# JialeTao/MRFA

Hardware: AMD Instinct MI355X
Metric: frames/sec (256x256 source+driving pair) fwd+bwd (higher is better)
Workload: dtype f32; 1 GPU; vox1.yaml MTIA (TokenPose_B) prior + DenseMotion + RaftFlow refinement, 256x256, bs=8/GPU, fwd+bwd+clip+Adam, train-mode BN, surrogate L1 loss; global_batch=8, parallelism=dp1, prior=mtia, background_predictor=False, sync_bn=False, launch=hipGraph, optimizer=FlatAdam (K20), mfma=bf16x6

## Files before the change

### mrfa_amd/build.py

```python
import glob
import os
import subprocess
import sys

HERE = os.path.dirname(os.path.abspath(__file__))
ROOT = os.path.dirname(HERE)
CSRC = os.path.join(HERE, "csrc")
LIBDIR = os.path.join(HERE, "_lib")
LIB = os.path.join(LIBDIR, "libmrfa_hip.so")
SOURCES = ["error.cpp", "conv_plan.hip", "conv_mfma.hip", "conv_split.hip", "conv_halo.hip", "conv_small.hip", "conv_lean.hip", "wgrad_mfma.hip", "wgrad_split.hip", "wgrad_halo.hip", "wgrad_small.hip", "wgrad_lean.hip", "conv_fewout.hip", "conv_fewout3.hip", "layout.hip", "pack_multi.hip", "norm.hip", "sample.hip", "elementwise.hip", "optim.hip", "tokenpose.hip", "attention_mfma.hip", "losses.hip", "prior.hip"]
FLAGS = ["--offload-arch=gfx950", "-O3", "-std=c++17", "-fPIC", "-I" + os.path.join(ROOT, "include"), "-I" + CSRC,
         "-Wno-unused-result"]


def _stale(out, deps):
    if not os.path.exists(out):
        return True
    t = os.path.getmtime(out)
    return any(os.path.getmtime(d) > t for d in deps)


def build(force: bool = False, verbose: bool = True) -> str:
    os.makedirs(LIBDIR, exist_ok=True)
    hipcc = os.environ.get("HIPCC", "/opt/rocm/bin/hipcc")
    headers = [os.path.join(ROOT, "include", "mrfa_hip.h")] + sorted(glob.glob(os.path.join(CSRC, "*.h")))
    objs = []
    procs = []
    for src in SOURCES:
        sp = os.path.join(CSRC, src)
        if not os.path.exists(sp):
            raise FileNotFoundError(sp)
        obj = os.path.join(LIBDIR, os.path.splitext(src)[0] + ".o")
        objs.append(obj)
        if force or _stale(obj, [sp] + headers):
            cmd = [hipcc] + FLAGS + (["-x", "hip"] if src.endswith(".cpp") else []) + ["-c", sp, "-o", obj]
            if verbose:
                print("[mrfa_amd.build]", " ".join(cmd), flush=True)
            procs.append((src, subprocess.Popen(cmd)))
    for src, pr in procs:
        if pr.wait() != 0:
            raise RuntimeError(f"hipcc failed on {src}")
    if force or _stale(LIB, objs):
        cmd = [hipcc, "--offload-arch=gfx950", "-shared", "-fPIC", "-o", LIB] + objs
        if verbose:
            print("[mrfa_amd.build]", " ".join(cmd), flush=True)
        subprocess.check_call(cmd)
    return LIB


if __name__ == "__main__":
    build(force="--force" in sys.argv)
    print(LIB)
```

### mrfa_amd/csrc/common.h

```cpp
#pragma once
#include <hip/hip_runtime.h>
#include <stdio.h>
#include <string.h>
#include "mrfa_hip.h"

typedef float f32x16 __attribute__((ext_vector_type(16)));
typedef float f32x4 __attribute__((ext_vector_type(4)));

void mrfa_set_error(const char* fmt, ...);

struct MrfaTuning {
    int conv_small_env;
    int conv_small;
    int conv_halo, conv_halo_min_tiles, conv_halo_pr, conv_halo_phase, conv_halo_bn256, conv_halo_bn192, conv_halo_bn64_fill;
    int conv_lean, conv_lean_min_wgs, conv_lean_geo, gemm_lean;
    int wgrad_halo, wgrad_halo_min_wgs, wgrad_halo_target_wgs, wgrad_halo_phase, wgrad_lean;
    int conv_fewout3, attention_mfma, split_target_256;
};
extern MrfaTuning g_tune;

struct HaloGeo { int PR, BN; bool phase; };

enum class ConvFamily { lean, gemm_lean, small, halo, halo_dgrad, rows_split, rows_f32, refused };
struct ConvPlan {
    ConvFamily family;
    char error[256];
    long long M;
    int KT;
    int lean_geo, gemm_cfg, small_tm, small_tn;
    HaloGeo halo;
    int BM, BN, splitk;
    bool w8;
    bool fused;
    bool fin_in_launch;
    bool reads_w;
    int last_config;
    bool groups_ok, bst_ok, stride2_ok, mask_ok, phase_dgrad_ok;
};
ConvPlan plan_conv(const mrfa_conv_params& p);

enum class WgradFamily { lean, small, halo, tiled, refused };
struct WgradPlan {
    WgradFamily family;
    char error[192];
    long long M;
    bool lean, small;
    bool groups_ok, stride2_ok;
};
WgradPlan plan_wgrad(const mrfa_wgrad_params& p);

int mrfa_conv_split_launch(hipStream_t st, const mrfa_conv_params& p, int KT, long long M, int splitk, int BN);
bool mrfa_conv_halo_eligible(const mrfa_conv_params& p, HaloGeo* geo);
int mrfa_conv_halo_launch(hipStream_t st, const mrfa_conv_params& p, const HaloGeo& geo);
int mrfa_wgrad_split_launch(hipStream_t st, const mrfa_wgrad_params& p, dim3 grid, long long M, long long kps, int tiles_n, int nsplit, int inner,
                            int total_splits, int taps, long long partial_stride, int BM, int BN);

bool mrfa_wgrad_halo_eligible(const mrfa_wgrad_params& p);
int mrfa_wgrad_halo_launch(hipStream_t st, const mrfa_wgrad_params& p);

bool mrfa_fewout3_wgrad(hipStream_t st, const float* x, int ldx, int N, int H, int W, int Cin, const float* dy, int lddy, int Cout, int R, int pad,
                        float* dw, float* dbias, int* rc);

int mrfa_conv_lean_pick(const mrfa_conv_params& p);
int mrfa_conv_lean_launch(hipStream_t st, const mrfa_conv_params& p, int geo);
int mrfa_gemm_lean_pick(const mrfa_conv_params& p, long long M);
int mrfa_gemm_lean_launch(hipStream_t st, const mrfa_conv_params& p, long long M, int cfg);

bool mrfa_conv_small_eligible(const mrfa_conv_params& p, long long M);
int mrfa_conv_small_launch(hipStream_t st, const mrfa_conv_params& p, long long M, int tm, int tn);

bool mrfa_attention_mfma_ok(int d, int n, const void* qkv, int ld, const void* out, int ldo, const void* dout, int lddo, const void* dqkv, int lddq);
int mrfa_attention_fwd_mfma(hipStream_t st, const float* qkv, int ld, int B, int n, int heads, int d, float scale, float* out, int ldo, float* lse);
int mrfa_attention_bwd_mfma(hipStream_t st, const float* qkv, int ld, const float* out, int ldo, const float* dout, int lddo, const float* lse,
                            float* delta, int B, int n, int heads, int d, float scale, float* dqkv, int lddq);

bool mrfa_wgrad_lean_eligible(const mrfa_wgrad_params& p);
int mrfa_wgrad_lean_multi(hipStream_t st, const mrfa_wgrad_params* ps, int n, unsigned char* taken);

bool mrfa_wgrad_small_eligible(const mrfa_wgrad_params& p, long long M);
int mrfa_wgrad_small_launch(hipStream_t st, const mrfa_wgrad_params& p, long long M);

#define MRFA_CHECK_ARG(cond, ...)                      \
    do {                                               \
        if (!(cond)) {                                 \
            mrfa_set_error(__VA_ARGS__);               \
            return 1;                                  \
        }                                              \
    } while (0)

#define MRFA_CHECK_LAUNCH(name)                                                   \
    do {                                                                          \
        hipError_t e_ = hipGetLastError();                                        \
        if (e_ != hipSuccess) {                                                   \
            mrfa_set_error("%s: launch failed: %s", name, hipGetErrorString(e_)); \
            return 2;                                                             \
        }                                                                         \
    } while (0)

static inline bool aligned16(const void* p) { return (reinterpret_cast<uintptr_t>(p) & 15u) == 0; }
static inline int cdiv(long long a, long long b) { return (int)((a + b - 1) / b); }

static inline int stream_grid(long long work_items, int block) {
    long long g = (work_items + block - 1) / block;
    if (g < 1) g = 1;
    if (g > 256 * 16) g = 256 * 16;
    return (int)g;
}

__device__ __forceinline__ int xcd_tile_index() {
    const int per_xcd = (int)gridDim.x >> 3;
    return (int)(blockIdx.x & 7) * per_xcd + (int)(blockIdx.x >> 3);
}

__device__ __forceinline__ void chain_prio() {
    __builtin_amdgcn_s_setprio(3);
}

__device__ __forceinline__ int stat_group(const mrfa_conv_params& p, long long row, long long M) {
    return p.groups > 1 ? (int)(row / (M / p.groups)) : 0;
}
__device__ __forceinline__ double* stat_slot(const mrfa_conv_params& p, int group, unsigned slot) {
    return p.stats + ((size_t)group * MRFA_STATS_SLOTS + slot % MRFA_STATS_SLOTS) * 2 * p.Cout;
}
static inline long long group_rows(const mrfa_conv_params& p, long long M) {
    if (p.groups <= 1) return M;
    return (p.N % p.groups) == 0 ? M / p.groups : 0;
}

__device__ __forceinline__ bool splitk_last_arriver(unsigned* ticket, unsigned nsplit) {
    __shared__ unsigned s_sk_ticket;
    asm volatile("s_waitcnt vmcnt(0)" ::: "memory");
    __syncthreads();
    if (threadIdx.x == 0) s_sk_ticket = __hip_atomic_fetch_add(ticket, 1u, __ATOMIC_RELAXED, __HIP_MEMORY_SCOPE_AGENT);
    __syncthreads();
    return s_sk_ticket == nsplit - 1;
}

__device__ __forceinline__ bool fin_last_arriver(unsigned* counter, unsigned participants, int idx) {
    __shared__ unsigned s_fin_ticket;
    asm volatile("s_waitcnt vmcnt(0)" ::: "memory");
    __syncthreads();
    if (threadIdx.x == 0) {
        if (idx < 0) {
            s_fin_ticket = __hip_atomic_fetch_add(counter, 1u, __ATOMIC_RELAXED, __HIP_MEMORY_SCOPE_AGENT) == participants - 1;
// ... 63 lines not shown
```

### mrfa_amd/csrc/conv_fewout.hip

```cpp
#include "common.h"

namespace {

constexpr int FT = 16;
constexpr int FCC = 16;
constexpr int FPS = FCC + 4;

template <int COUT, int PY, int RT>
__global__ __launch_bounds__(256) void conv_fewout_fwd_kernel(const float* __restrict__ x, int ldx, int H, int W, int Cin,
                                                             const float* __restrict__ w, const float* __restrict__ bias,
                                                             float* __restrict__ y, int ldy, int Ho, int Wo, int Rdyn, int pad,
                                                             int accumulate, int tiles_x, int tiles_y, int cper) {
    extern __shared__ __attribute__((aligned(16))) float smem[];
    const int R = RT > 0 ? RT : Rdyn;
    const int HTW = FT + R - 1, HTH = FT * PY + R - 1;
    const int tid = threadIdx.x;
    const int tx = tid & 15, ty = tid >> 4;
    const int bt = blockIdx.x;
    const int n = bt / (tiles_x * tiles_y);
    const int trem = bt - n * tiles_x * tiles_y;
    const int ty0 = (trem / tiles_x) * FT * PY, tx0 = (trem % tiles_x) * FT;
    const int T = R * R;
    float acc[PY][COUT];
#pragma unroll
// ... 145 lines not shown
                    const float* xrow = xs + ((py + r) * HT + s) * ps + g4 * 4;
                    const float* drow = dys + py * FT * 4;
#pragma unroll 4
                    for (int pxx = 0; pxx < FT; ++pxx) {
                        const f32x4 xv = *reinterpret_cast<const f32x4*>(xrow + pxx * ps);
                        const f32x4 dv = *reinterpret_cast<const f32x4*>(drow + pxx * 4);
#pragma unroll
                        for (int c = 0; c < COUT; ++c) acc[c] += xv * dv[c];
                    }
                }
            }
            if (dbias && c0 == 0 && tid < COUT) {
                float sacc = 0.f;
                for (int q = 0; q < 256; ++q) sacc += dys[q * 4 + tid];
                bsum += sacc;
            }
        }
        if (active) {
#pragma unroll
            for (int c = 0; c < COUT; ++c) {
                float* d = dw + ((size_t)c * T + tap) * Cin + c0 + g4 * 4;
#pragma unroll
                for (int q = 0; q < 4; ++q)
                    if (c0 + g4 * 4 + q < Cin) atomicAdd(d + q, acc[c][q]);
            }
        }
        if (dbias && c0 == 0 && tid < COUT) atomicAdd(dbias + tid, bsum);
    }
}

}

extern "C" int mrfa_conv_fewout_fwd(void* stream, const float* x, int ldx, int N, int H, int W, int Cin, const float* w,
                                    const float* bias, float* y, int ldy, int Cout, int R, int pad, int accumulate) {
    MRFA_CHECK_ARG(x && w && y && Cout >= 1 && Cout <= 4 && (Cin % 4) == 0 && (ldx % 4) == 0 && aligned16(x) && aligned16(w),
                   "conv_fewout_fwd: needs Cout <= 4, Cin %% 4 == 0, 16-B aligned x / w");
    const int Ho = H + 2 * pad - R + 1, Wo = W + 2 * pad - R + 1;
    const int PY = (R >= 5 && Cout <= 2 && Ho >= 32) ? 2 : 1;
    const bool rt7 = true;
    const int tiles_x = cdiv(Wo, FT), tiles_y = cdiv(Ho, FT * PY);
    const size_t lds = (size_t)(FT * PY + R - 1) * (FT + R - 1) * FPS * sizeof(float);
    if (lds > 64 * 1024) {
        MRFA_CHECK_ARG(lds <= 160 * 1024, "conv_fewout_fwd: halo tile does not fit the LDS");
    }
    hipStream_t st = (hipStream_t)stream;
    const int ntiles = N * tiles_x * tiles_y;
    const int chunks = cdiv(Cin, FCC);
    const int want = 1024;
    int csplit = 1;
    if (ntiles < want / 2 && chunks > 1) {
        csplit = cdiv(want, ntiles);
        if (csplit > chunks) csplit = chunks;
    }
    const int cper = cdiv(chunks, csplit) * FCC;
    csplit = cdiv(Cin, cper);
    if (csplit > 1 && !accumulate) {
        const long long tot = (long long)N * Ho * Wo * Cout;
        hipLaunchKernelGGL(fewout_init_kernel, dim3((unsigned)cdiv(tot, 256)), dim3(256), 0, st, y, ldy, (long long)N * Ho * Wo, Cout, bias);
    }
    dim3 grid((unsigned)ntiles, (unsigned)csplit);
#define FWD3(co, py, rt)                                                                                                                        \
    do {                                                                                                                                    \
        if (lds > 64 * 1024)                                                                                                                \
            (void)hipFuncSetAttribute(reinterpret_cast<const void*>(conv_fewout_fwd_kernel<co, py, rt>), hipFuncAttributeMaxDynamicSharedMemorySize, (int)lds); \
        hipLaunchKernelGGL((conv_fewout_fwd_kernel<co, py, rt>), grid, dim3(256), lds, st, x, ldx, H, W, Cin, w, bias, y, ldy, Ho, Wo, R, pad,   \
                           accumulate, tiles_x, tiles_y, cper);                                                                             \
    } while (0)
#define FWD2(co, py) do { if (R == 7 && rt7) FWD3(co, py, 7); else FWD3(co, py, 0); } while (0)
#define FWD(co) do { if (PY == 4) FWD2(co, 4); else if (PY == 2) FWD2(co, 2); else FWD2(co, 1); } while (0)
    switch (Cout) { case 1: FWD(1); break; case 2: FWD(2); break; case 3: FWD(3); break; default: FWD(4); break; }
#undef FWD
#undef FWD2
#undef FWD3
    MRFA_CHECK_LAUNCH("conv_fewout_fwd");
    return 0;
}

extern "C" int mrfa_conv_fewout_wgrad(void* stream, const float* x, int ldx, int N, int H, int W, int Cin, const float* dy, int lddy,
                                      int Cout, int R, int pad, float* dw, float* dbias) {
    MRFA_CHECK_ARG(x && dy && dw && Cout >= 1 && Cout <= 4 && (Cin % 4) == 0 && (ldx % 4) == 0 && aligned16(x),
                   "conv_fewout_wgrad: needs Cout <= 4, Cin %% 4 == 0, 16-B aligned x");
    {
        int rc3 = 0;
        if (mrfa_fewout3_wgrad((hipStream_t)stream, x, ldx, N, H, W, Cin, dy, lddy, Cout, R, pad, dw, dbias, &rc3)) return rc3;
    }
    const int Ho = H + 2 * pad - R + 1, Wo = W + 2 * pad - R + 1;
    const int tiles_x = cdiv(Wo, FT), tiles_y = cdiv(Ho, FT);
    const int ntiles = N * tiles_x * tiles_y;
    const int T = R * R;
    MRFA_CHECK_ARG(T * 1 <= 256, "conv_fewout_wgrad: kernel too large");
    int cc = 4;
    const int HT = FT + R - 1;
    auto lds_of = [&](int c) { return ((size_t)HT * HT * (c + 4) + 256 * 4) * sizeof(float); };
    const int cc_max = ntiles < 64 ? 16 : 64;
    while (cc * 2 <= cc_max && T * (cc * 2 / 4) <= 256 && cc * 2 <= ((Cin + 3) / 4 * 4) && lds_of(cc * 2) <= 64 * 1024) cc *= 2;
    const size_t lds = lds_of(cc);
    MRFA_CHECK_ARG(lds <= 64 * 1024, "conv_fewout_wgrad: LDS tile too large");
    dim3 grid((unsigned)(ntiles < 512 ? ntiles : 512), (unsigned)cdiv(Cin, cc));
    hipStream_t st = (hipStream_t)stream;
#define WG(co) hipLaunchKernelGGL((conv_fewout_wgrad_kernel<co>), grid, dim3(256), lds, st, x, ldx, H, W, Cin, dy, lddy, Ho, Wo, R, pad, dw, \
                                  dbias, tiles_x, tiles_y, ntiles, cc)
    switch (Cout) { case 1: WG(1); break; case 2: WG(2); break; case 3: WG(3); break; default: WG(4); break; }
#undef WG
    MRFA_CHECK_LAUNCH("conv_fewout_wgrad");
    return 0;
}
```

### mrfa_amd/csrc/conv_plan.hip

```cpp
#include "common.h"
#include <stdarg.h>
#include <stdlib.h>

namespace {
int env_int(const char* name, int dflt) { const char* e = getenv(name); return e ? atoi(e) : dflt; }
int env_on(const char* name) { const char* e = getenv(name); return !(e && e[0] == '0'); }
}

MrfaTuning g_tune = {
     env_on("MRFA_CONV_SMALL"),  1,
     env_on("MRFA_CONV_HALO"),  128,  0,  1,  1,
     1,  1,
     env_on("MRFA_CONV_LEAN"),  128,  -1,
     env_int("MRFA_GEMM_LEAN", 1),
     env_on("MRFA_WGRAD_HALO"),  192,  256,  1,
     env_on("MRFA_WGRAD_LEAN"),
     1,  env_on("MRFA_ATTENTION_MFMA"),  env_int("MRFA_SPLIT_TARGET_256", 1),
};

enum TuneKind { T_ON, T_INT, T_NONNEG, T_NONNEG_ON, T_LEVEL, T_POS };
static const struct { const char* key; int* field; TuneKind kind; } TUNING_KEYS[] = {
    {"conv_small", &g_tune.conv_small, T_ON},
    {"conv_halo", &g_tune.conv_halo, T_ON},
    {"conv_halo_min_tiles", &g_tune.conv_halo_min_tiles, T_INT},
    {"conv_halo_pr", &g_tune.conv_halo_pr, T_INT},
    {"conv_halo_phase", &g_tune.conv_halo_phase, T_ON},
    {"conv_halo_bn256", &g_tune.conv_halo_bn256, T_ON},
    {"conv_halo_bn192", &g_tune.conv_halo_bn192, T_ON},
    {"conv_halo_bn64_fill", &g_tune.conv_halo_bn64_fill, T_ON},
    {"conv_lean", &g_tune.conv_lean, T_ON},
    {"conv_lean_min_wgs", &g_tune.conv_lean_min_wgs, T_NONNEG},
    {"conv_lean_geo", &g_tune.conv_lean_geo, T_INT},
    {"gemm_lean", &g_tune.gemm_lean, T_LEVEL},
    {"wgrad_halo", &g_tune.wgrad_halo, T_ON},
    {"wgrad_halo_min_wgs", &g_tune.wgrad_halo_min_wgs, T_NONNEG},
    {"wgrad_halo_target_wgs", &g_tune.wgrad_halo_target_wgs, T_POS},
    {"wgrad_halo_phase", &g_tune.wgrad_halo_phase, T_NONNEG_ON},
    {"wgrad_lean", &g_tune.wgrad_lean, T_ON},
    {"conv_fewout3", &g_tune.conv_fewout3, T_ON},
    {"attention_mfma", &g_tune.attention_mfma, T_ON},
};

extern "C" int mrfa_set_tuning(const char* key, int value) {
    if (!key) return -1;
    for (const auto& k : TUNING_KEYS) {
        if (strcmp(key, k.key)) continue;
        const int prev = *k.field;
        switch (k.kind) {
            case T_ON: *k.field = value != 0; break;
            case T_INT: *k.field = value; break;
            case T_NONNEG: if (value >= 0) *k.field = value; break;
            case T_NONNEG_ON: if (value >= 0) *k.field = value != 0; break;
            case T_LEVEL: if (value >= 0) *k.field = value > 2 ? 2 : value; break;
            case T_POS: if (value > 0) *k.field = value; break;
        }
        return prev;
    }
    return -1;
}

namespace {
constexpr int BK = 32;

template <typename Plan>
Plan& refuse(Plan& c, const char* fmt, ...) {
    va_list ap;
    va_start(ap, fmt);
    vsnprintf(c.error, sizeof(c.error), fmt, ap);
    va_end(ap);
    c.family = decltype(c.family)::refused;
    return c;
}

void plan_rows(ConvPlan& c, const mrfa_conv_params& p, int mode) {
    const bool flat = p.kflat > 0;
    const long long M = c.M;
    const int KT = c.KT;
    const int nb = p.nbatch > 1 ? p.nbatch : 1;
    int BN = 128;
    {
        const int cands[4] = {128, 96, 64, 32};
        const double pen[4] = {1.0, 1.08, 1.16, 1.3};
        double best = 1e18;
        for (int i = 0; i < 4; ++i) {
            if (cands[i] == 96 && flat) continue;
            const double cost = (double)cdiv(p.Cout, cands[i]) * cands[i] * pen[i];
            if (cost < best) { best = cost; BN = cands[i]; }
        }
    }
    if (mode >= 1 && !flat && p.Cout >= 32) BN = p.Cout <= 64 ? 64 : 128;
    auto ntiles = [&](int bm, int bn) { return ((M + bm - 1) / bm) * cdiv(p.Cout, bn) * nb; };
    int BM = 128;
    if (BN == 96 && ntiles(128, 96) < 384) BN = 128;
    if (BN == 128) { if (M <= 32) BM = 32; else if (M <= 64) BM = 64; }
    else if (BN == 64 && M <= 64) BM = 64;
    int splitk = 1;
    const bool auto_split = (p.splitk == 0);
    if (p.splitk > 1) splitk = p.splitk;
    {
        const bool short_k_big_m = KT < 32 && M > 4096;
        const bool grouped_stats = p.groups > 1 && p.stats && !(p.sk_ticket && !p.accumulate);
        const int max_split = (auto_split && !short_k_big_m && !grouped_stats) ? (KT / 2 > 0 ? KT / 2 : 1) : 1;
        long long t = ntiles(BM, BN);
        if (t < 384 && !(short_k_big_m && t >= 128)) {
            const bool half_target = g_tune.split_target_256 && auto_split && p.sk_ticket && !p.accumulate && KT >= 72 && KT <= 320 && BM == 128 && t >= 8 && t <= 16;
            int want = (int)(((half_target ? 256 : 512) + t - 1) / t);
            if (auto_split) splitk = want <= max_split ? want : max_split;
            const int min_bm = (BN == 128) ? 32 : (BN == 64 ? 64 : 128);
            while (!half_target && ntiles(BM, BN) * splitk < 384 && BM > min_bm) {
                BM >>= 1;
                if (auto_split) {
                    t = ntiles(BM, BN);
                    want = (int)((512 + t - 1) / t);
                    splitk = want <= max_split ? want : max_split;
                }
            }
            if (splitk < 1) splitk = 1;
        }
    }
    bool w8 = false;
    if (p.tile) {
        BM = p.tile >> 16; BN = p.tile & 0x7fff; w8 = (p.tile & 0x8000) != 0;
// ... 23 lines not shown
    c.splitk = 1;
    c.reads_w = true;
    c.fin_in_launch = p.fin_scale != nullptr;

    c.lean_geo = flat ? -1 : mrfa_conv_lean_pick(p);
    c.gemm_cfg = (flat || c.lean_geo >= 0) ? -1 : mrfa_gemm_lean_pick(p, c.M);
    const bool lean = c.lean_geo >= 0, gemm = c.gemm_cfg >= 0;
    const bool small = !lean && !gemm && g_tune.conv_small_env && g_tune.conv_small && mrfa_conv_small_eligible(p, c.M);
    const bool halo = !flat && mrfa_conv_halo_eligible(p, &c.halo);

    const long long rows = group_rows(p, c.M);
    c.groups_ok = p.groups <= 1 || !(p.stats || p.fin_scale || p.bst_x || p.in_scale) ||
                  (p.nbatch <= 1 && p.splitk <= 1 && rows > 0 &&
                   (lean || gemm || (!p.in_scale && ((rows % 128) == 0 || small || (p.stride <= 1 && halo)))));
    c.bst_ok = p.stats && !p.fin_scale && p.stride >= 0 && !flat && (lean || gemm || small);
    c.stride2_ok = p.stride == 2 && p.Hout == (p.Hin + 2 * p.pad - p.R) / 2 + 1 && p.Wout == (p.Win + 2 * p.pad - p.S) / 2 + 1 &&
                   (flat ? (!p.ups && p.nbatch <= 1 && p.splitk <= 1 && p.ktab) : small);
    c.mask_ok = halo;
    c.phase_dgrad_ok = p.ups == 2 && halo;

    if (!(p.x && p.w)) return refuse(c, "conv2d: null pointer");
    if (!(p.N > 0 && p.Cin > 0 && p.Cout > 0 && p.Hout > 0 && p.Wout > 0)) return refuse(c, "conv2d: bad sizes");
    if (!(p.R >= 1 && p.S >= 1 && p.R <= 15 && p.S <= 15)) return refuse(c, "conv2d: kernel size %dx%d unsupported", p.R, p.S);
    if (!((p.w_ld % 4) == 0 && aligned16(p.w))) return refuse(c, "conv2d: packed weight must be 16-B aligned, w_ld %% 4 == 0");
    if (!flat && (p.Cin % 32) != 0) return refuse(c, "conv2d: chunked mode needs Cin %% 32 == 0 (got %d); use flat mode", p.Cin);
    if (!flat && !((p.ldx % 4) == 0 && aligned16(p.x))) return refuse(c, "conv2d: chunked mode needs 16-B aligned x and ldx %% 4 == 0");
    if (!flat && p.in_scale && !(aligned16(p.in_scale) && aligned16(p.in_shift))) return refuse(c, "conv2d: in_scale/in_shift alignment");
    if (flat && !(p.ktab != nullptr && aligned16(p.ktab))) return refuse(c, "conv2d: flat mode needs a 16-B aligned ktab");
    if (lean) {
        c.family = ConvFamily::lean;
        c.reads_w = false;
        c.last_config = (32 << 16) | (32 << 4) | 4 | (1 << 27);
        return c;
    }
    if (gemm) {
        c.family = ConvFamily::gemm_lean;
        c.reads_w = false;
        c.last_config = (64 << 16) | (64 << 4) | 4 | (1 << 26);
        return c;
    }
    if (small) {
        c.family = ConvFamily::small;
        const int ncols = (p.Cout + 15) / 16 * 16;
        auto waves = [&](int wm, int wn) { return ((c.M + wm - 1) / wm) * ((ncols + wn - 1) / wn); };
        int tm = 2, tn = 2;
        if (waves(32, 32) < 2048) { tm = 1; tn = 2; }
        if (tm == 1 && waves(16, 32) < 2048) { tn = 1; }
        if (ncols % 32 != 0 && tn == 2 && ncols < 32) tn = 1;
        if (p.groups > 1 && tm == 2 && (rows % 128) != 0) tm = 1;
        c.small_tm = tm;
        c.small_tn = tn;
        c.last_config = (16 << 16) | (16 << 4) | 8;
        return c;
    }
    if (p.stride < 0 || p.stride > 2 || (p.stride == 2 && !(flat && !p.ups && p.nbatch <= 1)))
        return refuse(c, "conv2d: stride = %d is only implemented by the one-wave-per-tile kernel and by flat-K launches: ask mrfa_conv2d_stride_supported() first", p.stride);
    if (p.mask && !halo) return refuse(c, "conv2d: `mask` is only honoured by the patch-tiled kernel: ask mrfa_conv2d_mask_supported() first");
    if (p.ups == 2 && !halo)
        return refuse(c, "conv2d: ups = 2 (phase data gradient of a fused-upsample layer) is only implemented for the shapes mrfa_conv2d_phase_dgrad_supported() reports");
    if (halo) {
        c.family = p.ups == 2 ? ConvFamily::halo_dgrad : ConvFamily::halo;
        c.reads_w = false;
        c.last_config = (128 << 16) | ((p.Cout <= 64 ? 64 : 128) << 4) | 4 | (1 << 28);
        return c;
    }
    plan_rows(c, p, mode);
    return c;
}

WgradPlan plan_wgrad(const mrfa_wgrad_params& p) {
    WgradPlan c = {};
    const bool flat = p.kflat > 0;
    c.M = (long long)p.N * p.Hout * p.Wout;
    c.lean = mrfa_wgrad_lean_eligible(p);
    c.small = g_tune.conv_small_env && g_tune.conv_small && mrfa_wgrad_small_eligible(p, c.M);
    c.groups_ok = p.groups <= 1 || !p.in_scale || c.lean;
    c.stride2_ok = p.stride == 2 && p.Hout == (p.Hin + 2 * p.pad - p.R) / 2 + 1 && p.Wout == (p.Win + 2 * p.pad - p.S) / 2 + 1 && c.small;
    if (!(p.x && p.dy && p.dw)) return refuse(c, "wgrad: null pointer");
    if (!flat && !((p.ldx % 4) == 0 && aligned16(p.x))) return refuse(c, "wgrad: x must be a 16-B aligned view with ld %% 4 == 0");
    if (flat && !p.ktab) return refuse(c, "wgrad: flat mode needs ktab");
    if (!(c.M < (1ll << 31) - 64)) return refuse(c, "wgrad: too many pixels");
    if (p.in_scale && c.lean) { c.family = WgradFamily::lean; return c; }
    if (!c.groups_ok) return refuse(c, "wgrad: groups = %d with a prologue is only implemented where mrfa_conv2d_wgrad_groups_supported() says so", p.groups);
    if (c.small) { c.family = WgradFamily::small; return c; }
    if (p.stride > 1) return refuse(c, "wgrad: stride = %d is only implemented by the small-problem kernel: ask mrfa_conv2d_wgrad_stride_supported() first", p.stride);
    c.family = !flat && mrfa_wgrad_halo_eligible(p) ? WgradFamily::halo : WgradFamily::tiled;
    return c;
}

extern "C" int mrfa_conv2d_split_k(const mrfa_conv_params* p) {
    if (!p) return 1;
    if (p->splitk > 1) return p->splitk;
    const ConvPlan c = plan_conv(*p);
    return c.family == ConvFamily::refused ? 1 : c.splitk;
}

extern "C" int mrfa_conv2d_reads_fp32_weights(const mrfa_conv_params* p) {
    if (!p) return 1;
    const ConvPlan c = plan_conv(*p);
    return c.family == ConvFamily::refused || c.reads_w ? 1 : 0;
}

extern "C" int mrfa_conv2d_groups_supported(const mrfa_conv_params* p) { return p && plan_conv(*p).groups_ok ? 1 : 0; }
extern "C" int mrfa_conv2d_bwdstats_supported(const mrfa_conv_params* p) { return p && plan_conv(*p).bst_ok ? 1 : 0; }
extern "C" int mrfa_conv2d_stride_supported(const mrfa_conv_params* p) { return p && plan_conv(*p).stride2_ok ? 1 : 0; }
extern "C" int mrfa_conv2d_mask_supported(const mrfa_conv_params* p) { return p && plan_conv(*p).mask_ok ? 1 : 0; }
extern "C" int mrfa_conv2d_phase_dgrad_supported(const mrfa_conv_params* p) { return p && plan_conv(*p).phase_dgrad_ok ? 1 : 0; }

extern "C" int mrfa_conv2d_wgrad_stride_supported(const mrfa_wgrad_params* p) { return p && plan_wgrad(*p).stride2_ok ? 1 : 0; }
extern "C" int mrfa_conv2d_wgrad_groups_supported(const mrfa_wgrad_params* p) { return p && plan_wgrad(*p).groups_ok ? 1 : 0; }
extern "C" int mrfa_conv2d_wgrad_lean_supported(const mrfa_wgrad_params* p) { return p && plan_wgrad(*p).lean ? 1 : 0; }
```

### mrfa_amd/csrc/wgrad_mfma.hip

```cpp
#include "common.h"
#include <stdlib.h>
#include <algorithm>

namespace {

constexpr int WBK = 32;
constexpr int KG = WBK / 4;

template <int BM, int BN, int WAVES_M, int WAVES_N, bool FLAT, bool ROWAL>
__global__ __launch_bounds__(WAVES_M * WAVES_N * 64) void wgrad_mfma_kernel(const mrfa_wgrad_params p, const long long M, const long long k_per_split,
                                                        const int tiles_n, const int nsplit, const int dy_scalar,
                                                        const int inner, const int total_splits, const int taps,
                                                        const long long partial_stride) {
    constexpr int WTM = BM / WAVES_M, WTN = BN / WAVES_N;
    constexpr int TM = WTM / 32, TN = WTN / 32;
    constexpr int NT = WAVES_M * WAVES_N * 64;
    static_assert((NT == 256 || NT == 512) && TM >= 1 && TN >= 1, "tile");
    constexpr int SA = BM / 4 + 4, SB = BN / 4 + 4;
    constexpr int PLA = 4 * SA, PLB = 4 * SB;
    constexpr int IA = (BM / 4) * KG, IB = (BN / 4) * KG;
    __shared__ f32x4 smem[2 * KG * (PLA + PLB)];

    const int tid = threadIdx.x, lane = tid & 63, wave = tid >> 6;
    const int wm = wave / WAVES_N, wn = wave % WAVES_N;
// ... 235 lines not shown
        const f32x4* Bs = smem + cur * KG * (PLA + PLB) + KG * PLA + b_lane;
#pragma unroll
        for (int q = 0; q < KG / 2; ++q) {
            f32x4 a[TM], b[TN];
#pragma unroll
            for (int i = 0; i < TM; ++i) a[i] = As[(2 * q + fh) * PLA + i * 8];
#pragma unroll
            for (int j = 0; j < TN; ++j) b[j] = Bs[(2 * q + fh) * PLB + j * 8];
#pragma unroll
            for (int e = 0; e < 4; ++e)
#pragma unroll
                for (int i = 0; i < TM; ++i)
#pragma unroll
                    for (int j = 0; j < TN; ++j)
                        acc[i][j] = __builtin_amdgcn_mfma_f32_32x32x2f32(a[i][e], b[j][e], acc[i][j], 0, 0, 0);
        }
        if (more) store_tiles(cur ^ 1);
        __syncthreads();
        cur ^= 1;
    }

#pragma unroll
    for (int j = 0; j < TN; ++j) {
        const int nn = ci0 + wn * WTN + j * 32 + (lane & 31);
        if (nn >= NTOT) continue;
        const int otap = FLAT ? nn / p.Cin : tap;
        const int ci = FLAT ? nn - otap * p.Cin : nn;
#pragma unroll
        for (int i = 0; i < TM; ++i) {
#pragma unroll
            for (int q = 0; q < 16; ++q) {
                const int co = co0 + wm * WTM + i * 32 + (q & 3) + 8 * (q >> 2) + 4 * fh;
                if (co < p.Cout) {
                    const size_t idx = ((size_t)otap * p.Cout + co) * p.Cin + ci;
                    if (partial_stride) p.ws[(size_t)split * partial_stride + idx] = acc[i][j][q] * p.alpha;
                    else atomicAdd(dw + idx, acc[i][j][q] * p.alpha);
                }
            }
        }
    }
    if (p.dbias != nullptr && tap == 0 && tile_n == 0) {
        float* red = reinterpret_cast<float*>(smem);
        __syncthreads();
        if (a_item) {
#pragma unroll
            for (int q = 0; q < 4; ++q) red[a_kg * BM + a_col + q] = bias_acc[q];
        }
        __syncthreads();
        if (tid < BM && co0 + tid < p.Cout) {
            float sacc = 0.f;
#pragma unroll
            for (int g = 0; g < KG; ++g) sacc += red[g * BM + tid];
            atomicAdd(p.dbias + co0 + tid, sacc);
        }
    }
}


__global__ void wgrad_reduce_kernel(const float* __restrict__ ws, float* __restrict__ dw, long long n, int nsplit) {
    const int groups = (nsplit + 15) / 16;
    const long long total = n * groups;
    for (long long t = blockIdx.x * (long long)blockDim.x + threadIdx.x; t < total; t += (long long)gridDim.x * blockDim.x) {
        const int g = (int)(t / n);
        const long long i = t - (long long)g * n;
        const int k0 = g * 16, k1 = min(nsplit, k0 + 16);
        float s = 0.f;
#pragma unroll 16
        for (int k = k0; k < k1; ++k) s += ws[(size_t)k * n + i];
        atomicAdd(dw + i, s);
    }
}

}

extern "C" int mrfa_conv2d_wgrad_nhwc(void* stream, const mrfa_wgrad_params* pp) {
    const mrfa_wgrad_params& p = *pp;
    hipStream_t st = (hipStream_t)stream;
    const WgradPlan c = plan_wgrad(p);
    const long long M = c.M;
    switch (c.family) {
        case WgradFamily::refused: mrfa_set_error("%s", c.error); return 1;
        case WgradFamily::lean: { unsigned char taken = 0; return mrfa_wgrad_lean_multi(st, &p, 1, &taken); }
        case WgradFamily::small: return mrfa_wgrad_small_launch(st, p, M);
        case WgradFamily::halo: return mrfa_wgrad_halo_launch(st, p);
        case WgradFamily::tiled: break;
    }
    const int dy_scalar = ((p.ldy % 4) == 0 && aligned16(p.dy) && (p.dy_bs % 4) == 0) ? 0 : 1;
    const bool flat = p.kflat > 0;
    const int nb = p.nbatch > 1 ? p.nbatch : 1;
    int taps = flat ? 1 : p.R * p.S;
    const int NTOT = flat ? p.kflat : p.Cin;
    auto pick = [](int n) {
        const int cands[4] = {128, 96, 64, 32};
        const double pen[4] = {1.0, 1.12, 1.35, 1.8};
        int best_t = 128;
        double best = 1e18;
        for (int i = 0; i < 4; ++i) {
            const double cost = (double)cdiv(n, cands[i]) * cands[i] * pen[i];
            if (cost < best) { best = cost; best_t = cands[i]; }
        }
        return best_t;
    };
    int BM = pick(p.Cout), BN = pick(NTOT);
    if (BM < 128 && BN < 128) {
        if (BM == 64 && BN == 64) {}
        else if (BM <= BN) BN = 128;
        else BM = 128;
    }
    if (flat && (BM == 96 || BN == 96)) { BM = BM == 96 ? 128 : BM; BN = BN == 96 ? 128 : BN; }
    const bool split_mode = mrfa_get_mfma_mode() >= 1 && !flat && (p.Wout % 8) == 0 && (M % WBK) == 0 && !dy_scalar && p.Cout >= 32 && NTOT >= 32;
    if (split_mode) { BM = p.Cout <= 64 ? 64 : 128; BN = NTOT <= 64 ? 64 : 128; if (BM == 64 && BN == 64) BN = 128; }
    int tiles_m = cdiv(p.Cout, BM), tiles_n = cdiv(NTOT, BN);
    int taps_arg = taps;
    constexpr bool cflat_on = true;
    if (cflat_on && split_mode && taps > 1 && (p.Cin % 4) == 0) {
        const double per_tap = (double)taps * tiles_n * BN * (BN == 64 ? 1.4 : 1.0), flat_w = (double)cdiv(taps * p.Cin, 128) * 128;
        if (flat_w <= 0.85 * per_tap) {
            BN = 128;
            tiles_n = cdiv(taps * p.Cin, 128);
            taps = 1;
            taps_arg = -1;
        }
    }
    const long long base = (long long)tiles_m * tiles_n * taps * nb;
    int nsplit = p.ksplit;
    if (nsplit <= 0) {
        const long long max_split = std::max<long long>(1, M / (8 * WBK));
        double best = 1e30;
        nsplit = 1;
        const long long inner_ = (long long)tiles_m * tiles_n * taps;
        for (long long ns = 1; ns <= std::min<long long>(max_split, 1024); ++ns) {
            const long long S = ns * nb;
            const long long ktiles = ((M + ns - 1) / ns + WBK - 1) / WBK;
            double rounds;
            if (S >= 8) rounds = (double)(((S + 7) / 8 * inner_ + 63) / 64);
            else rounds = (double)((S * inner_ + 511) / 512);
            const double cost = rounds * (double)(ktiles + 6);
            if (cost < best * 0.999) { best = cost; nsplit = (int)ns; }
        }
    }
    long long kps = (M + nsplit - 1) / nsplit;
    kps = (kps + WBK - 1) / WBK * WBK;
    nsplit = (int)((M + kps - 1) / kps);
    const int inner = tiles_m * tiles_n * taps;
    const int total_splits = nsplit * nb;
    const long long wn = (long long)(flat ? 1 : taps) * 0 + (long long)p.R * p.S * p.Cout * p.Cin;
    const long long partial_stride = (nb == 1 && nsplit >= 24 && p.ws && wn * nsplit * 4 <= p.ws_bytes) ? wn : 0;
    dim3 grid((unsigned)(cdiv(total_splits, 8) * 8 * inner));
    const bool rowal = (p.Wout % WBK) == 0;
#define WLAUNCH(bm, bn, wm, wn, fl, ra)                                                                                     \
    hipLaunchKernelGGL((wgrad_mfma_kernel<bm, bn, wm, wn, fl, ra>), grid, dim3((wm) * (wn) * 64), 0, st, p, M, kps, tiles_n, nsplit, dy_scalar, \
                       inner, total_splits, taps, partial_stride)
#define WCFG(bm, bn, wm, wn)                                              \
    if (BM == bm && BN == bn) {                                           \
        if (flat && rowal) WLAUNCH(bm, bn, wm, wn, true, true);           \
        else if (flat) WLAUNCH(bm, bn, wm, wn, true, false);              \
        else if (rowal) WLAUNCH(bm, bn, wm, wn, false, true);             \
        else WLAUNCH(bm, bn, wm, wn, false, false);                       \
    }
    if (split_mode) {
        const int rc = mrfa_wgrad_split_launch(st, p, grid, M, kps, tiles_n, nsplit, inner, total_splits, taps_arg, partial_stride, BM, BN);
        if (rc) return rc;
    }
    else if (BM == 128 && BN == 128 && !flat && rowal && !p.tile8_off) { WLAUNCH(128, 128, 2, 4, false, true); }
    else WCFG(128, 128, 2, 2)
    else WCFG(128, 64, 2, 2)
// ... 17 lines not shown
```

Measured before the change: 102.2 pairs/s.

## Add MFMA tap-GEMM weight-gradient kernel for few-channel convolutions

Adds a new kernel that computes weight gradients for convolutions with very few output channels (Cout<=4) or very few input channels (Cin 2-3, 3x3 or 7x7) as a small tap-by-channel GEMM on MFMA 16x16x4 f32. It stages pixel tiles of the wide tensor in shared memory with register prefetch of the next tile and reduces partial sums with atomics. It is wired ahead of the existing fewout3 path and into the wgrad planner as a new family, enabled by default. The aim is to replace poorly parallel scalar or tiled-GEMM paths for these skinny shapes, at the cost of heavy atomic traffic and a grid-size heuristic.

Result: no change. 102.0 pairs/s (-0.2%).

```diff
diff --git a/mrfa_amd/build.py b/mrfa_amd/build.py
--- a/mrfa_amd/build.py
+++ b/mrfa_amd/build.py
@@ -8,7 +8,7 @@
 CSRC = os.path.join(HERE, "csrc")
 LIBDIR = os.path.join(HERE, "_lib")
 LIB = os.path.join(LIBDIR, "libmrfa_hip.so")
-SOURCES = ["error.cpp", "conv_plan.hip", "conv_mfma.hip", "conv_split.hip", "conv_halo.hip", "conv_small.hip", "conv_lean.hip", "wgrad_mfma.hip", "wgrad_split.hip", "wgrad_halo.hip", "wgrad_small.hip", "wgrad_lean.hip", "conv_fewout.hip", "conv_fewout3.hip", "layout.hip", "pack_multi.hip", "norm.hip", "sample.hip", "elementwise.hip", "optim.hip", "tokenpose.hip", "attention_mfma.hip", "losses.hip", "prior.hip"]
+SOURCES = ["error.cpp", "conv_plan.hip", "conv_mfma.hip", "conv_split.hip", "conv_halo.hip", "conv_small.hip", "conv_lean.hip", "wgrad_mfma.hip", "wgrad_split.hip", "wgrad_halo.hip", "wgrad_small.hip", "wgrad_lean.hip", "conv_fewout.hip", "conv_fewout3.hip", "conv_fewch.hip", "layout.hip", "pack_multi.hip", "norm.hip", "sample.hip", "elementwise.hip", "optim.hip", "tokenpose.hip", "attention_mfma.hip", "losses.hip", "prior.hip"]
 FLAGS = ["--offload-arch=gfx950", "-O3", "-std=c++17", "-fPIC", "-I" + os.path.join(ROOT, "include"), "-I" + CSRC,
          "-Wno-unused-result"]
 
diff --git a/mrfa_amd/csrc/common.h b/mrfa_amd/csrc/common.h
--- a/mrfa_amd/csrc/common.h
+++ b/mrfa_amd/csrc/common.h
@@ -16,6 +16,7 @@
     int conv_lean, conv_lean_min_wgs, conv_lean_geo, gemm_lean;
     int wgrad_halo, wgrad_halo_min_wgs, wgrad_halo_target_wgs, wgrad_halo_phase, wgrad_lean;
     int conv_fewout3, attention_mfma, split_target_256;
+    int conv_fewch;
 };
 extern MrfaTuning g_tune;
 
@@ -39,7 +40,7 @@
 };
 ConvPlan plan_conv(const mrfa_conv_params& p);
 
-enum class WgradFamily { lean, small, halo, tiled, refused };
+enum class WgradFamily { lean, small, fewch, halo, tiled, refused };
 struct WgradPlan {
     WgradFamily family;
     char error[192];
@@ -60,6 +61,11 @@
 
 bool mrfa_fewout3_wgrad(hipStream_t st, const float* x, int ldx, int N, int H, int W, int Cin, const float* dy, int lddy, int Cout, int R, int pad,
                         float* dw, float* dbias, int* rc);
+
+bool mrfa_fewch_wgrad_fewout(hipStream_t st, const float* x, int ldx, int N, int H, int W, int Cin, const float* dy, int lddy, int Cout, int R, int pad,
+                             float* dw, float* dbias, int* rc);
+bool mrfa_fewch_wgrad_fewin_takes(const mrfa_wgrad_params& p);
+int mrfa_fewch_wgrad_fewin_launch(hipStream_t st, const mrfa_wgrad_params& p);
 
 int mrfa_conv_lean_pick(const mrfa_conv_params& p);
 int mrfa_conv_lean_launch(hipStream_t st, const mrfa_conv_params& p, int geo);
diff --git a/mrfa_amd/csrc/conv_fewch.hip b/mrfa_amd/csrc/conv_fewch.hip
--- /dev/null
+++ b/mrfa_amd/csrc/conv_fewch.hip
@@ -0,0 +1,216 @@
+#include "common.h"
+
+namespace {
+
+constexpr int PW = 16, PH = 4;
+
+struct FewchArgs {
+    const float* big; int ldb, BH, BW, CB;
+    const float* tiny; int ldt, SH, SW;
+    int org;
+    int center;
+    float* dw; float* dbias; float alpha;
+    int tiles_x, tiles_y, ntiles;
+};
+
+template <int FEW, int R, int NBW, bool FEWIN>
+__global__ __launch_bounds__(256) void fewch_wgrad_kernel(const FewchArgs a) {
+    constexpr int T = R * R, ROWS = T * FEW, MB = (ROWS + (FEWIN ? 1 : 0) + 15) / 16;
+    constexpr int CS = 64 * NBW, PS = CS + 16, G4 = CS / 4, LD = PW * PH * G4 / 256;
+    constexpr int TW = PW + R - 1, TH = PH + R - 1;
+    __shared__ __attribute__((aligned(16))) float xs[PW * PH * PS];
+    __shared__ float ts[TH * TW * FEW];
+    const int tid = threadIdx.x, lane = tid & 63, wave = tid >> 6;
+    const int m16 = lane & 15, k4 = lane >> 4;
+    const int c0 = blockIdx.y * CS;
+    const int CB = a.CB;
+    const bool wave_on = c0 + wave * NBW * 16 < CB;
+
+    int aoff[MB];
+#pragma unroll
+    for (int mb = 0; mb < MB; ++mb) {
+        const int row = mb * 16 + m16 < ROWS ? mb * 16 + m16 : 0;
+        const int tap = row / FEW, f = row - tap * FEW;
+        const int r = tap / R, s = tap - r * R;
+        aoff[mb] = FEWIN ? (r * TW + s) * FEW + f : ((R - 1 - r) * TW + (R - 1 - s)) * FEW + f;
+    }
+    f32x4 acc[MB][NBW];
+#pragma unroll
+    for (int mb = 0; mb < MB; ++mb)
+#pragma unroll
+        for (int j = 0; j < NBW; ++j) acc[mb][j] = f32x4{0.f, 0.f, 0.f, 0.f};
+    float bsum[FEW];
+#pragma unroll
+    for (int c = 0; c < FEW; ++c) bsum[c] = 0.f;
+
+    const int tiles_img = a.tiles_x * a.tiles_y;
+    f32x4 pre[LD];
+    auto fetch = [&](int t) {
+        const int n = t / tiles_img;
+        const int trem = t - n * tiles_img;
+        const int y0 = (trem / a.tiles_x) * PH, x0 = (trem % a.tiles_x) * PW;
+        const float* bin = a.big + (size_t)n * a.BH * a.BW * a.ldb;
+#pragma unroll
+        for (int j = 0; j < LD; ++j) {
+            const int i = tid + j * 256;
+            const int g = i % G4, pix = i / G4;
+            const int iy = y0 + pix / PW, ix = x0 + pix % PW;
+            const bool ok = iy < a.BH && ix < a.BW && c0 + g * 4 < CB;
+            const f32x4 v = *reinterpret_cast<const f32x4*>(bin + (ok ? ((size_t)iy * a.BW + ix) * a.ldb + c0 + g * 4 : (size_t)0));
+            pre[j] = ok ? v : f32x4{0.f, 0.f, 0.f, 0.f};
+        }
+    };
+    if ((int)blockIdx.x < a.ntiles) fetch(blockIdx.x);
+    for (int t = blockIdx.x; t < a.ntiles; t += gridDim.x) {
+        const int n = t / tiles_img;
+        const int trem = t - n * tiles_img;
+        const int y0 = (trem / a.tiles_x) * PH, x0 = (trem % a.tiles_x) * PW;
+        __syncthreads();
+#pragma unroll
+        for (int j = 0; j < LD; ++j) {
+            const int i = tid + j * 256;
+            *reinterpret_cast<f32x4*>(xs + (i / G4) * PS + (i % G4) * 4) = pre[j];
+        }
+        {
+            const float* tin = a.tiny + (size_t)n * a.SH * a.SW * a.ldt;
+            const int ty0 = y0 + a.org, tx0 = x0 + a.org;
+            for (int i = tid; i < TH * TW * FEW; i += 256) {
+                const int f = i % FEW, tp = i / FEW;
+                const int sy = ty0 + tp / TW, sx = tx0 + tp % TW;
+                const bool ok = (unsigned)sy < (unsigned)a.SH && (unsigned)sx < (unsigned)a.SW;
+                const float v = tin[ok ? ((size_t)sy * a.SW + sx) * a.ldt + f : (size_t)0];
+                ts[i] = ok ? v : 0.f;
+            }
+        }
+        __syncthreads();
+        if (t + (int)gridDim.x < a.ntiles) fetch(t + gridDim.x);
+        if (wave_on) {
+#pragma unroll 4
+            for (int ks = 0; ks < PW * PH / 4; ++ks) {
+                const int py = ks >> 2, px = (ks & 3) * 4 + k4;
+                const float* ap = ts + (py * TW + px) * FEW;
+                const float* bp = xs + (ks * 4 + k4) * PS + wave * NBW * 16 + m16;
+                float b[NBW];
+#pragma unroll
+                for (int j = 0; j < NBW; ++j) b[j] = bp[j * 16];
+#pragma unroll
+                for (int mb = 0; mb < MB; ++mb) {
+                    float av = ap[aoff[mb]];
+                    if (FEWIN && mb == ROWS / 16) av = m16 == ROWS % 16 ? 1.f : av;
+#pragma unroll
+                    for (int j = 0; j < NBW; ++j) acc[mb][j] = __builtin_amdgcn_mfma_f32_16x16x4f32(av, b[j], acc[mb][j], 0, 0, 0);
+                }
+            }
+        }
+        if (!FEWIN && a.dbias && blockIdx.y == 0 && tid < PW * PH) {
+            const float* dp = ts + (((tid / PW) + a.center) * TW + (tid % PW) + a.center) * FEW;
+#pragma unroll
+            for (int c = 0; c < FEW; ++c) bsum[c] += dp[c];
+        }
+    }
+    if (wave_on) {
+#pragma unroll
+        for (int mb = 0; mb < MB; ++mb)
+#pragma unroll
+            for (int j = 0; j < NBW; ++j) {
+                const int col = c0 + (wave * NBW + j) * 16 + m16;
+#pragma unroll
+                for (int i = 0; i < 4; ++i) {
+                    const int row = mb * 16 + k4 * 4 + i;
+                    const int tap = row / FEW, f = row - tap * FEW;
+                    if (col < CB) {
+                        if (FEWIN) {
+                            if (row < ROWS) atomicAdd(a.dw + ((size_t)tap * CB + col) * FEW + f, acc[mb][j][i] * a.alpha);
+                            else if (row == ROWS && a.dbias) atomicAdd(a.dbias + col, acc[mb][j][i]);
+                        } else if (row < ROWS) {
+                            atomicAdd(a.dw + ((size_t)f * T + tap) * CB + col, acc[mb][j][i]);
+                        }
+                    }
+                }
+            }
+    }
+    if (!FEWIN && a.dbias && blockIdx.y == 0 && wave == 0) {
+#pragma unroll
+        for (int c = 0; c < FEW; ++c) {
+            const float s = wave_sum(bsum[c]);
+            if (lane == 0) atomicAdd(a.dbias + c, s);
+        }
+    }
+}
+
+struct FewchGrid { int nbw; dim3 grid; };
+FewchGrid fewch_grid(int ntiles, int CB, int cap) {
+    const int nbw = (CB > 64 && (long long)ntiles * cdiv(CB, 128) >= 256) ? 2 : 1;
+    const int slices = cdiv(CB, 64 * nbw);
+    long long tot = (long long)ntiles * slices / 8;
+    if (tot < 256) tot = 256;
+    if (tot > cap) tot = cap;
+    int gx = (int)(tot / slices);
+    if (gx < 1) gx = 1;
+    if (gx > ntiles) gx = ntiles;
+    return FewchGrid{nbw, dim3((unsigned)gx, (unsigned)slices)};
+}
+
+bool fewout_takes(const float* x, int ldx, int N, int H, int W, int Cin, int Cout, int R, int pad) {
+    return (R == 3 || R == 7) && Cout >= 1 && Cout <= 4 && Cin >= 4 && (Cin % 4) == 0 && (ldx % 4) == 0 && aligned16(x) && pad >= 0 && 2 * pad <= R - 1 &&
+           H + 2 * pad - R + 1 >= 1 && W + 2 * pad - R + 1 >= 1 && (long long)N * cdiv(W, PW) * cdiv(H, PH) < (1ll << 30);
+}
+
+}
+
+bool mrfa_fewch_wgrad_fewout(hipStream_t st, const float* x, int ldx, int N, int H, int W, int Cin, const float* dy, int lddy, int Cout, int R, int pad,
+                             float* dw, float* dbias, int* rc) {
+    *rc = 0;
+    if (!g_tune.conv_fewch) return false;
+    if (!fewout_takes(x, ldx, N, H, W, Cin, Cout, R, pad)) {
+        if (g_tune.conv_fewch < 2) return false;
+        mrfa_set_error("conv_fewout_wgrad: conv_fewch = 2, but the tap-GEMM kernel does not take Cin %d Cout %d R %d pad %d ldx %d", Cin, Cout, R, pad, ldx);
+        *rc = 1;
+        return true;
+    }
+    FewchArgs a = {};
+    a.big = x; a.ldb = ldx; a.BH = H; a.BW = W; a.CB = Cin;
+    a.tiny = dy; a.ldt = lddy; a.SH = H + 2 * pad - R + 1; a.SW = W + 2 * pad - R + 1;
+    a.org = pad - (R - 1); a.center = R - 1 - pad;
+    a.dw = dw; a.dbias = dbias; a.alpha = 1.f;
+    a.tiles_x = cdiv(W, PW); a.tiles_y = cdiv(H, PH); a.ntiles = N * a.tiles_x * a.tiles_y;
+    const FewchGrid g = fewch_grid(a.ntiles, Cin, 768);
+#define FEWCH_WG3(co, r, nb) hipLaunchKernelGGL((fewch_wgrad_kernel<co, r, nb, false>), g.grid, dim3(256), 0, st, a)
+#define FEWCH_WG2(co, r) do { if (g.nbw == 2) FEWCH_WG3(co, r, 2); else FEWCH_WG3(co, r, 1); } while (0)
+#define FEWCH_WG(co) do { if (R == 3) FEWCH_WG2(co, 3); else FEWCH_WG2(co, 7); } while (0)
+    switch (Cout) { case 1: FEWCH_WG(1); break; case 2: FEWCH_WG(2); break; case 3: FEWCH_WG(3); break; default: FEWCH_WG(4); break; }
+#undef FEWCH_WG
+#undef FEWCH_WG2
+#undef FEWCH_WG3
+    if (hipGetLastError() != hipSuccess) {
+        mrfa_set_error("conv_fewout_wgrad(tap GEMM): launch failed");
+        *rc = 2;
+    }
+    return true;
+}
+
+bool mrfa_fewch_wgrad_fewin_takes(const mrfa_wgrad_params& p) {
+    return p.kflat > 0 && (p.Cin == 2 || p.Cin == 3) && p.R == p.S && (p.R == 3 || p.R == 7) && p.stride <= 1 && p.ups == 0 && !p.in_scale && p.nbatch <= 1 &&
+           p.Cout >= 16 && (p.Cout % 4) == 0 && (p.ldy % 4) == 0 && aligned16(p.dy) && p.ldx >= p.Cin && p.pad >= 0 && p.N > 0 && p.Hout > 0 && p.Wout > 0 &&
+           p.Hout == p.Hin + 2 * p.pad - p.R + 1 && p.Wout == p.Win + 2 * p.pad - p.S + 1 &&
+           (long long)p.N * cdiv(p.Wout, PW) * cdiv(p.Hout, PH) < (1ll << 30);
+}
+
+int mrfa_fewch_wgrad_fewin_launch(hipStream_t st, const mrfa_wgrad_params& p) {
+    FewchArgs a = {};
+    a.big = p.dy; a.ldb = p.ldy; a.BH = p.Hout; a.BW = p.Wout; a.CB = p.Cout;
+    a.tiny = p.x; a.ldt = p.ldx; a.SH = p.Hin; a.SW = p.Win;
+    a.org = -p.pad; a.center = 0;
+    a.dw = p.dw; a.dbias = p.dbias; a.alpha = p.alpha;
+    a.tiles_x = cdiv(p.Wout, PW); a.tiles_y = cdiv(p.Hout, PH); a.ntiles = p.N * a.tiles_x * a.tiles_y;
+    const FewchGrid g = fewch_grid(a.ntiles, p.Cout, 512);
+#define FEWCH_WI3(ci, r, nb) hipLaunchKernelGGL((fewch_wgrad_kernel<ci, r, nb, true>), g.grid, dim3(256), 0, st, a)
+#define FEWCH_WI2(ci, r) do { if (g.nbw == 2) FEWCH_WI3(ci, r, 2); else FEWCH_WI3(ci, r, 1); } while (0)
+#define FEWCH_WI(ci) do { if (p.R == 3) FEWCH_WI2(ci, 3); else FEWCH_WI2(ci, 7); } while (0)
+    if (p.Cin == 2) FEWCH_WI(2); else FEWCH_WI(3);
+#undef FEWCH_WI
+#undef FEWCH_WI2
+#undef FEWCH_WI3
+    MRFA_CHECK_LAUNCH("mrfa_conv2d_wgrad_nhwc(tap GEMM)");
+    return 0;
+}
diff --git a/mrfa_amd/csrc/conv_fewout.hip b/mrfa_amd/csrc/conv_fewout.hip
--- a/mrfa_amd/csrc/conv_fewout.hip
+++ b/mrfa_amd/csrc/conv_fewout.hip
@@ -251,6 +251,7 @@
                    "conv_fewout_wgrad: needs Cout <= 4, Cin %% 4 == 0, 16-B aligned x");
     {
         int rc3 = 0;
+        if (mrfa_fewch_wgrad_fewout((hipStream_t)stream, x, ldx, N, H, W, Cin, dy, lddy, Cout, R, pad, dw, dbias, &rc3)) return rc3;
         if (mrfa_fewout3_wgrad((hipStream_t)stream, x, ldx, N, H, W, Cin, dy, lddy, Cout, R, pad, dw, dbias, &rc3)) return rc3;
     }
     const int Ho = H + 2 * pad - R + 1, Wo = W + 2 * pad - R + 1;
diff --git a/mrfa_amd/csrc/conv_plan.hip b/mrfa_amd/csrc/conv_plan.hip
--- a/mrfa_amd/csrc/conv_plan.hip
+++ b/mrfa_amd/csrc/conv_plan.hip
@@ -16,6 +16,7 @@
      env_on("MRFA_WGRAD_HALO"),  192,  256,  1,
      env_on("MRFA_WGRAD_LEAN"),
      1,  env_on("MRFA_ATTENTION_MFMA"),  env_int("MRFA_SPLIT_TARGET_256", 1),
+     1,
 };
 
 enum TuneKind { T_ON, T_INT, T_NONNEG, T_NONNEG_ON, T_LEVEL, T_POS };
@@ -38,6 +39,7 @@
     {"wgrad_halo_phase", &g_tune.wgrad_halo_phase, T_NONNEG_ON},
     {"wgrad_lean", &g_tune.wgrad_lean, T_ON},
     {"conv_fewout3", &g_tune.conv_fewout3, T_ON},
+    {"conv_fewch", &g_tune.conv_fewch, T_LEVEL},
     {"attention_mfma", &g_tune.attention_mfma, T_ON},
 };
 
@@ -227,9 +229,17 @@
     if (!(c.M < (1ll << 31) - 64)) return refuse(c, "wgrad: too many pixels");
     if (p.in_scale && c.lean) { c.family = WgradFamily::lean; return c; }
     if (!c.groups_ok) return refuse(c, "wgrad: groups = %d with a prologue is only implemented where mrfa_conv2d_wgrad_groups_supported() says so", p.groups);
+    const bool fewch = g_tune.conv_fewch && mrfa_fewch_wgrad_fewin_takes(p);
+    if (g_tune.conv_fewch == 2 && flat && p.Cin <= 3) {
+        if (!fewch) return refuse(c, "wgrad: conv_fewch = 2, but the tap-GEMM kernel does not take %d->%d %dx%d stride %d", p.Cin, p.Cout, p.R, p.S, p.stride);
+        c.small = false;
+        c.family = WgradFamily::fewch;
+        return c;
+    }
     if (c.small) { c.family = WgradFamily::small; return c; }
     if (p.stride > 1) return refuse(c, "wgrad: stride = %d is only implemented by the small-problem kernel: ask mrfa_conv2d_wgrad_stride_supported() first", p.stride);
-    c.family = !flat && mrfa_wgrad_halo_eligible(p) ? WgradFamily::halo : WgradFamily::tiled;
+    if (fewch) { c.family = WgradFamily::fewch; return c; }
+    c.family =!flat && mrfa_wgrad_halo_eligible(p) ? WgradFamily::halo : WgradFamily::tiled;
     return c;
 }
 
diff --git a/mrfa_amd/csrc/wgrad_mfma.hip b/mrfa_amd/csrc/wgrad_mfma.hip
--- a/mrfa_amd/csrc/wgrad_mfma.hip
+++ b/mrfa_amd/csrc/wgrad_mfma.hip
@@ -341,6 +341,7 @@
         case WgradFamily::refused: mrfa_set_error("%s", c.error); return 1;
         case WgradFamily::lean: { unsigned char taken = 0; return mrfa_wgrad_lean_multi(st, &p, 1, &taken); }
         case WgradFamily::small: return mrfa_wgrad_small_launch(st, p, M);
+        case WgradFamily::fewch: return mrfa_fewch_wgrad_fewin_launch(st, p);
         case WgradFamily::halo: return mrfa_wgrad_halo_launch(st, p);
         case WgradFamily::tiled: break;
     }
```
